# masafumiendo/benchnav

Hardware: AMD Instinct MI355X
Metric: MPPI solve-steps/sec (K=1024,T=50,256x256 map) (higher is better)
Workload: dtype f32

## Files before the change

### benchnav_amd/csrc/rollout_sampled.hip

```cpp
#include "mppi_device.h"

namespace bn {

namespace {

constexpr int kSampledWaves = 8;
constexpr int kSampledThreads = 64 * kSampledWaves;

__host__ __device__ inline size_t sampled_lds_floats(int T, int WN)
{
    const size_t TP = (size_t)((T + 2) & ~1);
    return 4 * 64 * (size_t)(T + 1) + 2 * (size_t)WN * WN + 2 * 64 * TP + 2 * (size_t)T * kUPad + 4 * (size_t)T + 128;
}

template <int EPS, int GEO, bool STORE_U>
__global__ __launch_bounds__(kSampledThreads) void rollout_sampled_kernel(const SolveParams p)
{
    extern __shared__ __attribute__((aligned(16))) float smem[];
    const int T = p.T, K = p.K, WN2 = p.WN * p.WN;
    const int TP = (T + 2) & ~1;
    float4 *XL = reinterpret_cast<float4 *>(smem);
    float2 *win2 = reinterpret_cast<float2 *>(smem + 4 * 64 * (T + 1));
    float *Zt = reinterpret_cast<float *>(win2 + WN2), *Zc = Zt + 64 * TP;
    float *Ul = Zc + 64 * TP, *ml = Ul + 2 * T * kUPad, *mv = ml + 2 * T, *el = mv + 2 * T, *ad = el + 64;
    const WgId wg = decode_wg(p);
    if (wg.idle) return;
    const int tid = threadIdx.x, lane = tid & 63, b = wg.b;
    if (wg.aux) {
        if (p.overlap) finish_body<GEO, true, kSampledThreads, false, true>(p, b, nullptr, p.cost_prev, p.state_prev, smem);
        else finish_body<GEO, true, kSampledThreads>(p, b, nullptr, p.cost_prev, p.state_prev, smem);
        return;
    }
    const int wid = __builtin_amdgcn_readfirstlane(tid >> 6);
    const int k = wg.blk * 64 + lane;
    const bool active = k < K;
    const int kk = active ? k : K - 1;
    const float *__restrict__ mu = p.map + (size_t)b * p.map_stride;
    const float *__restrict__ sg = p.slip_std + (size_t)b * p.map_stride;
    const float sx = p.state[b * 3 + 0], sy = p.state[b * 3 + 1], sth = p.state[b * 3 + 2];
    const float gx = p.goal[b * 2 + 0], gy = p.goal[b * 2 + 1];
    const Win w = window_origin<GEO>(p, sx, sy);
    const size_t Kp = (size_t)p.Kp;
    float *Xb = p.X + (size_t)b * (T + 1) * 3 * Kp + k;
    float *Ub = STORE_U ? p.U + (size_t)b * T * 2 * Kp + k : nullptr;

    BN_STAMP(0);
    for (int e = tid; e < WN2; e += kSampledThreads) {
        const int r = e / p.WN, c = e - r * p.WN;
        const size_t g = (size_t)min(w.wy0 + r, p.G - 1) * p.G + min(w.wx0 + c, p.G - 1);
        win2[e] = make_float2(mu[g], sg[g]);
    }
    const bool ovs = p.overlap != 0;
    const bool tpub = p.flag_part != nullptr;
    if (!ovs)
    for (int j = tid; j < 2 * T; j += kSampledThreads) {
        const float m = p.mean[(size_t)b * 2 * T + j];
        ml[j] = m;
        mv[j] = m * ((j & 1) ? p.iv1 : p.iv0);
    }
    if (wg.blk == 0 && tid < 3) { if (tpub) store_agent(p.state_copy + b * 3 + tid, p.state[b * 3 + tid]); else p.state_copy[b * 3 + tid] = p.state[b * 3 + tid]; }
    if (p.state_snap && wg.blk == 0 && tid < 3) p.state_snap[b * 3 + tid] = p.state[b * 3 + tid];
    __syncthreads();

    {
        const int nE = (T + 1) >> 1, nS = TP >> 1;
        for (int q = nE + wid; q < nE + nS; q += kSampledWaves) {
            {
                const int r0 = 2 * (q - nE), r1 = r0 + 1;
                float z[4];
                if (p.zt) {
                    z[0] = r0 < T ? p.zt[((size_t)b * T + r0) * K + kk] : 0.0f;
                    z[1] = r1 < T ? p.zt[((size_t)b * T + r1) * K + kk] : 0.0f;
                    z[2] = r0 <= T ? p.zc[((size_t)b * (T + 1) + r0) * K + kk] : 0.0f;
                    z[3] = r1 <= T ? p.zc[((size_t)b * (T + 1) + r1) * K + kk] : 0.0f;
                } else {
                    philox_slip_block(p.seed, p.solve, (uint32_t)b, (uint32_t)(kk + p.k0), (uint32_t)(q - nE), z);
                }
                Zt[r0 * 64 + lane] = z[0]; Zt[r1 * 64 + lane] = z[1];
                Zc[r0 * 64 + lane] = z[2]; Zc[r1 * 64 + lane] = z[3];
            }
        }
        if (ovs) {
            if (tid == 0) wait_counter<16>(flag_ctr(p.flag_part, p.prev_slot * p.B + b), p.wait_part, p);
            __syncthreads();
            for (int j = tid; j < 2 * T; j += kSampledThreads) {
                const float m = load_agent(p.mean + (size_t)b * 2 * T + j);
                ml[j] = m;
                mv[j] = m * ((j & 1) ? p.iv1 : p.iv0);
            }
            __syncthreads();
        }
        if (p.mean_snap && wg.blk == 0 && wid == 0) snapshot_mean(p, b, ml, lane);
        for (int q = wid; q < nE; q += kSampledWaves) produce_pair<EPS, STORE_U>(p, p.eps, b, kk, 2 * q, p.solve, ml, Ul, Ub, Kp, lane);
    }
    __syncthreads();
    BN_STAMP(1);

    if (wid == 0) {
        SlipChain c;
        c.x = sx; c.y = sy; c.th = sth;
        sincos_spec(c.th, c.sn, c.cs);
        c.e = slip_cell_safe<GEO, true>(p, w, sx, sy);
        float xn, yn, tn;
        slip_chain_step<GEO, true>(p, win2, w, c, Ul[lane], Ul[kUPad + lane], Zt[lane], xn, yn, tn);
        XL[lane] = make_float4(xn, yn, tn, __int_as_float(c.e));
        int t = 1;
        for (; t + 4 <= T; t += 4) {
            float uq[4][3];
#pragma unroll
            for (int i = 0; i < 4; ++i) {
                uq[i][0] = Ul[(2 * (t + i)) * kUPad + lane]; uq[i][1] = Ul[(2 * (t + i) + 1) * kUPad + lane];
                uq[i][2] = Zt[(t + i) * 64 + lane];
            }
#pragma unroll
            for (int i = 0; i < 4; ++i) {
                slip_chain_step<GEO, false>(p, win2, w, c, uq[i][0], uq[i][1], uq[i][2], xn, yn, tn);
                __builtin_amdgcn_sched_barrier(0);
                XL[(t + i) * 64 + lane] = make_float4(xn, yn, tn, __int_as_float(c.e));
            }
        }
        for (; t < T; ++t) {
            slip_chain_step<GEO, false>(p, win2, w, c, Ul[(2 * t) * kUPad + lane], Ul[(2 * t + 1) * kUPad + lane], Zt[t * 64 + lane],
                                        xn, yn, tn);
            XL[t * 64 + lane] = make_float4(xn, yn, tn, __int_as_float(c.e));
        }
        XL[T * 64 + lane] = make_float4(c.x, c.y, c.th, __int_as_float(c.e));
    } else if (wid == 1) {
        double Ad = 0.0;
        for (int t = 0; t < T; ++t)
            Ad += (double)(p.lambda_ * (mv[2 * t] * Ul[(2 * t) * kUPad + lane] + mv[2 * t + 1] * Ul[(2 * t + 1) * kUPad + lane]));
        ad[lane] = (float)Ad;
    }
    __syncthreads();
    BN_STAMP(2);

    for (int t = wid; t <= T; t += kSampledWaves) {
        const float4 o = XL[t * 64 + lane];
        float *Xt = Xb + (size_t)(3 * t) * Kp;
        Xt[0] = o.x; Xt[Kp] = o.y; Xt[2 * Kp] = o.z;
        const float2 ms = win2[__float_as_int(o.w)];
        const float tc = trav_from_slip(ms.x, ms.y, Zc[t * 64 + lane]);
        const float dx = o.x - gx, dy = o.y - gy;
        Zc[t * 64 + lane] = sqrt_cr_normal(dx * dx + dy * dy) + (tc <= p.thr ? 1.0e4f : 0.0f);
    }
    __syncthreads();
    BN_STAMP(3);

    if (wid == 0) {
        double Sd = 0.0;
#pragma unroll 16
        for (int t = 0; t < T; ++t) Sd += (double)Zc[t * 64 + lane];
        const float cost = ((float)Sd + Zc[T * 64 + lane]) + ad[lane];
        if (active) { if (tpub) store_agent(p.cost + (size_t)b * K + k, cost); else p.cost[(size_t)b * K + k] = cost; }
        const float zz = active ? (-cost) / p.lambda_ : -INFINITY;
        const float zmax = wave_max(zz);
        const float e = active ? expf(zz - zmax) : 0.0f;
        const float esum = wave_sum(e);
        el[lane] = e;
        if (lane == 0) {
            float *part = p.part + ((size_t)b * p.nblk + wg.blk) * (2 + 2 * T);
            store_agent(part, zmax); store_agent(part + 1, esum);
        }
    }
    __syncthreads();
    column_sums<kSampledThreads, true>(Ul, el, T, tid, p.part + ((size_t)b * p.nblk + wg.blk) * (2 + 2 * T));
    BN_STAMP(5);
    if (p.ustar_cur) ticket_merge<kSampledThreads>(p, b, wg.blk, smem);
}

template <int EPS, int GEO, bool STORE_U>
__global__ __launch_bounds__(64) void rollout_sampled_global_kernel(const SolveParams p)
{
    extern __shared__ __attribute__((aligned(16))) float smem[];
    const int T = p.T, K = p.K;
    float *ml = smem, *mv = ml + 2 * T, *Ul = mv + 2 * T, *el = Ul + 2 * T * kUPad;
    const WgId wg = decode_wg(p);
    if (wg.idle) return;
    const int lane = threadIdx.x, b = wg.b;
    const int k = wg.blk * 64 + lane;
    const bool active = k < K;
    const int kk = active ? k : K - 1;
    const float *__restrict__ mu = p.map + (size_t)b * p.map_stride;
    const float *__restrict__ sg = p.slip_std + (size_t)b * p.map_stride;
    const float sx = p.state[b * 3 + 0], sy = p.state[b * 3 + 1], sth = p.state[b * 3 + 2];
    const float gx = p.goal[b * 2 + 0], gy = p.goal[b * 2 + 1];
    const Win w{0, 0, 0.f, 0.f, 0.f, 0.f};
    for (int j = lane; j < 2 * T; j += 64) {
        const float m = p.mean[(size_t)b * 2 * T + j];
        ml[j] = m;
        mv[j] = m * ((j & 1) ? p.iv1 : p.iv0);
    }
    if (wg.blk == 0 && lane < 3) p.state_copy[b * 3 + lane] = p.state[b * 3 + lane];
    if (p.state_snap && wg.blk == 0 && lane < 3) p.state_snap[b * 3 + lane] = p.state[b * 3 + lane];
    __syncthreads();
    const size_t Kp = (size_t)p.Kp;
    float *Xb = p.X + (size_t)b * (T + 1) * 3 * Kp + k;
    float *Ub = STORE_U ? p.U + (size_t)b * T * 2 * Kp + k : nullptr;
    for (int t = 0; t < T; t += 2) produce_pair<EPS, STORE_U>(p, p.eps, b, kk, t, p.solve, ml, Ul, Ub, Kp, lane);
    __syncthreads();
    float x = sx, y = sy, th = sth;
    float sn, cs;
    sincos_spec(th, sn, cs);
    float zq[4] = {0.f, 0.f, 0.f, 0.f};
    double Sd = 0.0, Ad = 0.0;
    for (int t = 0; t < T; ++t) {
        if (p.zt) {
            zq[t & 1] = p.zt[((size_t)b * T + t) * K + kk];
            zq[2 + (t & 1)] = p.zc[((size_t)b * (T + 1) + t) * K + kk];
        } else if ((t & 1) == 0) {
            philox_slip_block(p.seed, p.solve, (uint32_t)b, (uint32_t)(kk + p.k0), (uint32_t)(t >> 1), zq);
        }
        const float u0 = Ul[(2 * t) * kUPad + lane], u1 = Ul[(2 * t + 1) * kUPad + lane];
        const int e = slip_cell_safe<GEO, false>(p, w, x, y);
        const float trav = trav_from_slip(mu[e], sg[e], zq[t & 1]);
        float xn, yn, tn;
        if (p.ref_order) {
            sincos_spec(th, sn, cs);
            const float tv = trav * u0;
            xn = x + (tv * cs) * p.dt; yn = y + (tv * sn) * p.dt;
            tn = th + (trav * u1) * p.dt;
            th = wrap_angle(tn);
        } else {
            const float g = u0 * p.dt, dth = trav * (u1 * p.dt);
            xn = __builtin_fmaf(trav, g * cs, x); yn = __builtin_fmaf(trav, g * sn, y);
            tn = theta_step(th, dth, t == 0);
            rotate_spec(cs, sn, dth);
        }
        float *Xt = Xb + (size_t)(3 * t) * Kp;
        Xt[0] = xn; Xt[Kp] = yn; Xt[2 * Kp] = tn;
        x = clampf(xn, p.x0, p.x_hi); y = clampf(yn, p.y0, p.y_hi);
        const int ec = slip_cell_safe<GEO, false>(p, w, xn, yn);
        const float tc = trav_from_slip(mu[ec], sg[ec], zq[2 + (t & 1)]);
        const float dx = xn - gx, dy = yn - gy;
        Sd += (double)(sqrt_cr_normal(dx * dx + dy * dy) + (tc <= p.thr ? 1.0e4f : 0.0f));
        Ad += (double)(p.lambda_ * (mv[2 * t] * u0 + mv[2 * t + 1] * u1));
    }
    {
        float *Xt = Xb + (size_t)(3 * T) * Kp;
        Xt[0] = x; Xt[Kp] = y; Xt[2 * Kp] = th;
    }
    if (p.zt) zq[2 + (T & 1)] = p.zc[((size_t)b * (T + 1) + T) * K + kk];
    else if ((T & 1) == 0) philox_slip_block(p.seed, p.solve, (uint32_t)b, (uint32_t)(kk + p.k0), (uint32_t)(T >> 1), zq);
    const int eT = slip_cell_safe<GEO, false>(p, w, x, y);
    const float tT = trav_from_slip(mu[eT], sg[eT], zq[2 + (T & 1)]);
    const float dxT = x - gx, dyT = y - gy;
    const float term = sqrt_cr_normal(dxT * dxT + dyT * dyT) + (tT <= p.thr ? 1.0e4f : 0.0f);
    const float cost = ((float)Sd + term) + (float)Ad;
    if (active) p.cost[(size_t)b * K + k] = cost;
    const float zz = active ? (-cost) / p.lambda_ : -INFINITY;
    const float zmax = wave_max(zz);
    const float e = active ? expf(zz - zmax) : 0.0f;
    const float esum = wave_sum(e);
    el[lane] = e;
    __syncthreads();
    float *part = p.part + ((size_t)b * p.nblk + wg.blk) * (2 + 2 * T);
    column_sums<64, false>(Ul, el, T, lane, part);
    if (lane == 0) { part[0] = zmax; part[1] = esum; }
}

__global__ void philox_slip_kernel(float *__restrict__ zt, float *__restrict__ zc, float *__restrict__ zo, uint64_t seed,
                                   uint64_t solve, int b, int K, int T, int k0)
{
    const int nS = ((T + 2) & ~1) >> 1;
    const size_t tot = (size_t)K * nS;
    for (size_t i = blockIdx.x * (size_t)blockDim.x + threadIdx.x; i < tot; i += (size_t)gridDim.x * blockDim.x) {
        const int k = (int)(i / nS), j = (int)(i - (size_t)k * nS);
        float z[4];
        philox_slip_block(seed, solve, (uint32_t)b, (uint32_t)(k + k0), (uint32_t)j, z);
        for (int s = 0; s < 2; ++s) {
            const int r = 2 * j + s;
            if (r < T) zt[(size_t)k * T + r] = z[s];
            if (r <= T) zc[(size_t)k * (T + 1) + r] = z[2 + s];
        }
    }
    if (blockIdx.x == 0)
        for (int j = threadIdx.x; 4 * j < T; j += blockDim.x) {
            float z[4];
            philox_slip_block(seed, solve, (uint32_t)b, 0xffffffffu, (uint32_t)j, z);
            for (int s = 0; s < 4; ++s)
                if (4 * j + s < T) zo[4 * j + s] = z[s];
        }
}


}

size_t sampled_resident_per_cu(const SolveParams &p)
{
    const size_t need = sizeof(float) * sampled_lds_floats(p.T, p.WN);
    return std::max<size_t>(1, std::min<size_t>(160 * 1024 / std::max<size_t>(need, 1), 32 / kSampledWaves));
}

bool sampled_fused(const SolveParams &p)
{
    const size_t need = sizeof(float) * sampled_lds_floats(p.T, p.WN);
    const size_t tail = finish_lds_bytes(p) + sizeof(float) * 64;
    return p.slip_on && !p.ref_order && p.WN > 0 && need <= 160 * 1024 && tail <= need && p.nblk <= 1024;
}


namespace {

template <int EPS, int GEO>
hipError_t launch_sampled_g(const SolveParams &p, hipStream_t s)
{
    const size_t lds_w = sizeof(float) * sampled_lds_floats(p.T, p.WN);
    const dim3 grid = rollout_grid(p, sampled_fused(p) && p.have_prev);
    if (sampled_fused(p)) {
#define BN_SL(SU)                                                                                                      \
    do { hipError_t e = ensure_lds(rollout_sampled_kernel<EPS, GEO, SU>, lds_w); if (e != hipSuccess) return e;        \
         rollout_sampled_kernel<EPS, GEO, SU><<<grid, dim3(kSampledThreads), lds_w, s>>>(p); } while (0)
        if (p.U) BN_SL(true); else BN_SL(false);
#undef BN_SL
    } else {
        const size_t lds = sizeof(float) * (4 * (size_t)p.T + 2 * (size_t)p.T * kUPad + 64);
#define BN_SL(SU)                                                                                                      \
    do { hipError_t e = ensure_lds(rollout_sampled_global_kernel<EPS, GEO, SU>, lds); if (e != hipSuccess) return e;   \
         rollout_sampled_global_kernel<EPS, GEO, SU><<<grid, dim3(64), lds, s>>>(p); } while (0)
        if (p.U) BN_SL(true); else BN_SL(false);
#undef BN_SL
    }
    return hipGetLastError();
}

template <int EPS>
hipError_t launch_sampled_e(const SolveParams &p, hipStream_t s)
{
    switch (geo_of(p)) {
    case kGeoPow2Origin0: return launch_sampled_g<EPS, kGeoPow2Origin0>(p, s);
    case kGeoPow2: return launch_sampled_g<EPS, kGeoPow2>(p, s);
    default: return launch_sampled_g<EPS, kGeoGeneral>(p, s);
    }
}


}

hipError_t launch_rollout_sampled(const SolveParams &p, EpsMode mode, hipStream_t s)
{
    switch (mode) {
    case kEpsPhilox: return launch_sampled_e<kEpsPhilox>(p, s);
    case kEpsKT2: return launch_sampled_e<kEpsKT2>(p, s);
    default: return launch_sampled_e<kEpsT2K>(p, s);
    }
}

hipError_t launch_philox_slip(float *zt, float *zc, float *zo, uint64_t seed, uint64_t solve, int b, int K, int T, int k0, hipStream_t s)
{
    philox_slip_kernel<<<grid_for((size_t)K * (T / 2 + 1)), 256, 0, s>>>(zt, zc, zo, seed, solve, b, K, T, k0);
    return hipGetLastError();
}


}
```

Baseline: 105,800.

## Pipeline sampled rollout stages with LDS progress flags instead of block barriers

Replaces the barrier-separated phases of the sampled rollout kernel with wave-specialized producer/consumer pipelining. Progress counters live in LDS: control chunks are computed in parallel and published, the serial slip chain starts as soon as its first chunk is ready, and other waves stream X writes and per-step cost accumulation behind the chain rather than waiting for it to finish. Noise generation is also split from the mean-dependent clamp, so it can proceed before the overlap wait for the new mean. This shortens the critical path around the serial chain but adds spin-waiting, volatile LDS polling and fragile memory ordering.

```diff
diff --git a/benchnav_amd/csrc/rollout_sampled.hip b/benchnav_amd/csrc/rollout_sampled.hip
--- a/benchnav_amd/csrc/rollout_sampled.hip
+++ b/benchnav_amd/csrc/rollout_sampled.hip
@@ -6,6 +6,33 @@
 
 constexpr int kSampledWaves = 8;
 constexpr int kSampledThreads = 64 * kSampledWaves;
+constexpr int kSampledTail = 4;
+
+typedef __attribute__((address_space(3))) volatile int lds_vint;
+
+__device__ __forceinline__ void post_progress(int *word, int v)
+{
+    asm volatile("" ::: "memory");
+    if ((threadIdx.x & 63) == 0) *(lds_vint *)word = v;
+}
+template <int SLEEP>
+__device__ __forceinline__ int wait_progress(int *word, int need)
+{
+    lds_vint *p3 = (lds_vint *)word;
+    int v;
+    while ((v = *p3) < need) __builtin_amdgcn_s_sleep(SLEEP);
+    asm volatile("" ::: "memory");
+    return __builtin_amdgcn_readfirstlane(v);
+}
+constexpr int kSampledProducers = kSampledWaves - 1;
+__device__ __forceinline__ bool controls_complete(int *prog, int nchunk, int lane)
+{
+    const int w = lane & (kSampledWaves - 1);
+    const int last = w == 0 ? 1 : w < nchunk ? w + ((nchunk - 1 - w) / kSampledProducers) * kSampledProducers + 1 : 0;
+    const int v = *(lds_vint *)(prog + 8 + w);
+    asm volatile("" ::: "memory");
+    return __builtin_amdgcn_ballot_w64(v < last) == 0;
+}
 
 __host__ __device__ inline size_t sampled_lds_floats(int T, int WN)
 {
@@ -23,6 +50,7 @@
     float2 *win2 = reinterpret_cast<float2 *>(smem + 4 * 64 * (T + 1));
     float *Zt = reinterpret_cast<float *>(win2 + WN2), *Zc = Zt + 64 * TP;
     float *Ul = Zc + 64 * TP, *ml = Ul + 2 * T * kUPad, *mv = ml + 2 * T, *el = mv + 2 * T, *ad = el + 64;
+    int *prog = reinterpret_cast<int *>(Zt + 64 * T);
     const WgId wg = decode_wg(p);
     if (wg.idle) return;
     const int tid = threadIdx.x, lane = tid & 63, b = wg.b;
@@ -60,13 +88,16 @@
     }
     if (wg.blk == 0 && tid < 3) { if (tpub) store_agent(p.state_copy + b * 3 + tid, p.state[b * 3 + tid]); else p.state_copy[b * 3 + tid] = p.state[b * 3 + tid]; }
     if (p.state_snap && wg.blk == 0 && tid < 3) p.state_snap[b * 3 + tid] = p.state[b * 3 + tid];
-    __syncthreads();
-
+    if (tid < 8 + kSampledWaves) prog[tid] = 0;
+    __syncthreads();
+
+    const int nchunk = (T + 3) >> 2;
+    const int cstep = wid == 0 ? nchunk : kSampledProducers;
     {
-        const int nE = (T + 1) >> 1, nS = TP >> 1;
-        for (int q = nE + wid; q < nE + nS; q += kSampledWaves) {
+        const int nS = TP >> 1;
+        for (int q = kSampledWaves - 1 - wid; q < nS; q += kSampledWaves) {
             {
-                const int r0 = 2 * (q - nE), r1 = r0 + 1;
+                const int r0 = 2 * q, r1 = r0 + 1;
                 float z[4];
                 if (p.zt) {
                     z[0] = r0 < T ? p.zt[((size_t)b * T + r0) * K + kk] : 0.0f;
@@ -74,27 +105,58 @@
                     z[2] = r0 <= T ? p.zc[((size_t)b * (T + 1) + r0) * K + kk] : 0.0f;
                     z[3] = r1 <= T ? p.zc[((size_t)b * (T + 1) + r1) * K + kk] : 0.0f;
                 } else {
-                    philox_slip_block(p.seed, p.solve, (uint32_t)b, (uint32_t)(kk + p.k0), (uint32_t)(q - nE), z);
+                    philox_slip_block(p.seed, p.solve, (uint32_t)b, (uint32_t)(kk + p.k0), (uint32_t)q, z);
                 }
-                Zt[r0 * 64 + lane] = z[0]; Zt[r1 * 64 + lane] = z[1];
+                if (r0 < T) Zt[r0 * 64 + lane] = z[0];
+                if (r1 < T) Zt[r1 * 64 + lane] = z[1];
                 Zc[r0 * 64 + lane] = z[2]; Zc[r1 * 64 + lane] = z[3];
             }
         }
+        for (int c = wid; c < nchunk; c += cstep)
+            for (int t = 4 * c; t < min(4 * c + 4, T); t += 2) {
+                float e[4];
+                noise_pair<EPS>(p, b, kk, t, e);
+                Ul[(2 * t) * kUPad + lane] = e[0];
+                Ul[(2 * t + 1) * kUPad + lane] = e[1];
+                if (t + 1 < T) { Ul[(2 * t + 2) * kUPad + lane] = e[2]; Ul[(2 * t + 3) * kUPad + lane] = e[3]; }
+            }
         if (ovs) {
             if (tid == 0) wait_counter<16>(flag_ctr(p.flag_part, p.prev_slot * p.B + b), p.wait_part, p);
+            BN_STAMP(13);
             __syncthreads();
             for (int j = tid; j < 2 * T; j += kSampledThreads) {
                 const float m = load_agent(p.mean + (size_t)b * 2 * T + j);
                 ml[j] = m;
                 mv[j] = m * ((j & 1) ? p.iv1 : p.iv0);
             }
-            __syncthreads();
-        }
-        if (p.mean_snap && wg.blk == 0 && wid == 0) snapshot_mean(p, b, ml, lane);
-        for (int q = wid; q < nE; q += kSampledWaves) produce_pair<EPS, STORE_U>(p, p.eps, b, kk, 2 * q, p.solve, ml, Ul, Ub, Kp, lane);
+        }
     }
     __syncthreads();
     BN_STAMP(1);
+
+    for (int c = wid; c < nchunk; c += cstep) {
+        const int t0 = 4 * c;
+        if (t0 + 4 <= T) {
+            float z[8], m[8];
+#pragma unroll
+            for (int i = 0; i < 8; ++i) { z[i] = Ul[(2 * t0 + i) * kUPad + lane]; m[i] = ml[2 * t0 + i]; }
+#pragma unroll
+            for (int i = 0; i < 8; ++i) {
+                const float u = (i & 1) ? clampf(m[i] + p.sigma1 * z[i], p.umin1, p.umax1) : clampf(m[i] + p.sigma0 * z[i], p.umin0, p.umax0);
+                Ul[(2 * t0 + i) * kUPad + lane] = u;
+                if (STORE_U) Ub[(size_t)(2 * t0 + i) * Kp] = u;
+            }
+        } else {
+            for (int t = t0; t < T; ++t) {
+                const float u0 = clampf(ml[2 * t] + p.sigma0 * Ul[(2 * t) * kUPad + lane], p.umin0, p.umax0);
+                const float u1 = clampf(ml[2 * t + 1] + p.sigma1 * Ul[(2 * t + 1) * kUPad + lane], p.umin1, p.umax1);
+                Ul[(2 * t) * kUPad + lane] = u0;
+                Ul[(2 * t + 1) * kUPad + lane] = u1;
+                if (STORE_U) { float *Ut = Ub + (size_t)(2 * t) * Kp; Ut[0] = u0; Ut[Kp] = u1; }
+            }
+        }
+        post_progress(prog + 8 + wid, c + 1);
+    }
 
     if (wid == 0) {
         SlipChain c;
@@ -102,55 +164,97 @@
         sincos_spec(c.th, c.sn, c.cs);
         c.e = slip_cell_safe<GEO, true>(p, w, sx, sy);
         float xn, yn, tn;
+        BN_WSTAMP(0);
+        bool all = controls_complete(prog, nchunk, lane);
         slip_chain_step<GEO, true>(p, win2, w, c, Ul[lane], Ul[kUPad + lane], Zt[lane], xn, yn, tn);
         XL[lane] = make_float4(xn, yn, tn, __int_as_float(c.e));
+        while (!all) { all = controls_complete(prog, nchunk, lane); if (!all) __builtin_amdgcn_s_sleep(1); }
         int t = 1;
-        for (; t + 4 <= T; t += 4) {
-            float uq[4][3];
-#pragma unroll
-            for (int i = 0; i < 4; ++i) {
-                uq[i][0] = Ul[(2 * (t + i)) * kUPad + lane]; uq[i][1] = Ul[(2 * (t + i) + 1) * kUPad + lane];
-                uq[i][2] = Zt[(t + i) * 64 + lane];
-            }
-#pragma unroll
-            for (int i = 0; i < 4; ++i) {
-                slip_chain_step<GEO, false>(p, win2, w, c, uq[i][0], uq[i][1], uq[i][2], xn, yn, tn);
-                __builtin_amdgcn_sched_barrier(0);
-                XL[(t + i) * 64 + lane] = make_float4(xn, yn, tn, __int_as_float(c.e));
-            }
-        }
+#define BN_SCHUNK(POSTALL)                                                                                             \
+        {                                                                                                              \
+            float uq[4][3];                                                                                            \
+            _Pragma("unroll") for (int i = 0; i < 4; ++i) {                                                            \
+                uq[i][0] = Ul[(2 * (t + i)) * kUPad + lane]; uq[i][1] = Ul[(2 * (t + i) + 1) * kUPad + lane];          \
+                uq[i][2] = Zt[(t + i) * 64 + lane];                                                                    \
+            }                                                                                                          \
+            _Pragma("unroll") for (int i = 0; i < 4; ++i) {                                                            \
+                slip_chain_step<GEO, false>(p, win2, w, c, uq[i][0], uq[i][1], uq[i][2], xn, yn, tn);                  \
+                __builtin_amdgcn_sched_barrier(0);                                                                     \
+                XL[(t + i) * 64 + lane] = make_float4(xn, yn, tn, __int_as_float(c.e));                                \
+                if ((POSTALL) || i == 3) post_progress(prog, t + i + 1);                                               \
+            }                                                                                                          \
+        }
+        for (; t + 4 <= T - kSampledTail; t += 4) BN_SCHUNK(false)
+        for (; t + 4 <= T; t += 4) BN_SCHUNK(true)
+#undef BN_SCHUNK
         for (; t < T; ++t) {
             slip_chain_step<GEO, false>(p, win2, w, c, Ul[(2 * t) * kUPad + lane], Ul[(2 * t + 1) * kUPad + lane], Zt[t * 64 + lane],
                                         xn, yn, tn);
             XL[t * 64 + lane] = make_float4(xn, yn, tn, __int_as_float(c.e));
+            post_progress(prog, t + 1);
         }
         XL[T * 64 + lane] = make_float4(c.x, c.y, c.th, __int_as_float(c.e));
+        post_progress(prog, T + 1);
+        BN_STAMP(2);
     } else if (wid == 1) {
+        while (!controls_complete(prog, nchunk, lane)) __builtin_amdgcn_s_sleep(1);
         double Ad = 0.0;
         for (int t = 0; t < T; ++t)
             Ad += (double)(p.lambda_ * (mv[2 * t] * Ul[(2 * t) * kUPad + lane] + mv[2 * t + 1] * Ul[(2 * t + 1) * kUPad + lane]));
         ad[lane] = (float)Ad;
-    }
-    __syncthreads();
-    BN_STAMP(2);
-
-    for (int t = wid; t <= T; t += kSampledWaves) {
-        const float4 o = XL[t * 64 + lane];
-        float *Xt = Xb + (size_t)(3 * t) * Kp;
-        Xt[0] = o.x; Xt[Kp] = o.y; Xt[2 * Kp] = o.z;
-        const float2 ms = win2[__float_as_int(o.w)];
-        const float tc = trav_from_slip(ms.x, ms.y, Zc[t * 64 + lane]);
-        const float dx = o.x - gx, dy = o.y - gy;
-        Zc[t * 64 + lane] = sqrt_cr_normal(dx * dx + dy * dy) + (tc <= p.thr ? 1.0e4f : 0.0f);
-    }
-    __syncthreads();
-    BN_STAMP(3);
-
-    if (wid == 0) {
+        post_progress(prog + 1, 1);
+    } else if (wid == 4) {
+        if (p.mean_snap && wg.blk == 0) snapshot_mean(p, b, ml, lane);
+    } else if (wid != 5) {
+        const int sw = (wid & 1) | ((wid >> 2) << 1);
+        int have = 0;
+        for (int t0 = 4 * sw; t0 <= T; t0 += 16) {
+            const int n = min(4, T + 1 - t0);
+            if (have < t0 + n) have = wait_progress<2>(prog, t0 + n);
+            float *Xt = Xb + (size_t)(3 * t0) * Kp;
+            if (n == 4) {
+                float4 o[4];
+#pragma unroll
+                for (int i = 0; i < 4; ++i) o[i] = XL[(t0 + i) * 64 + lane];
+#pragma unroll
+                for (int i = 0; i < 4; ++i) { Xt[(size_t)(3 * i) * Kp] = o[i].x; Xt[(size_t)(3 * i + 1) * Kp] = o[i].y; Xt[(size_t)(3 * i + 2) * Kp] = o[i].z; }
+            } else {
+                for (int i = 0; i < n; ++i) {
+                    const float4 o = XL[(t0 + i) * 64 + lane];
+                    Xt[(size_t)(3 * i) * Kp] = o.x; Xt[(size_t)(3 * i + 1) * Kp] = o.y; Xt[(size_t)(3 * i + 2) * Kp] = o.z;
+                }
+            }
+        }
+    } else {
+        auto stage = [&](const float4 o, const float z) {
+            const float2 ms = win2[__float_as_int(o.w)];
+            const float tc = trav_from_slip(ms.x, ms.y, z);
+            const float dx = o.x - gx, dy = o.y - gy;
+            return sqrt_cr_normal(dx * dx + dy * dy) + (tc <= p.thr ? 1.0e4f : 0.0f);
+        };
         double Sd = 0.0;
-#pragma unroll 16
-        for (int t = 0; t < T; ++t) Sd += (double)Zc[t * 64 + lane];
-        const float cost = ((float)Sd + Zc[T * 64 + lane]) + ad[lane];
+        float term = 0.0f;
+        int done = 0;
+        while (done <= T) {
+            const int have = wait_progress<1>(prog, done + 1);
+            for (; done + 4 <= min(have, T); done += 4) {
+                float4 o[4];
+                float z[4], s[4];
+#pragma unroll
+                for (int i = 0; i < 4; ++i) { o[i] = XL[(done + i) * 64 + lane]; z[i] = Zc[(done + i) * 64 + lane]; }
+#pragma unroll
+                for (int i = 0; i < 4; ++i) s[i] = stage(o[i], z[i]);
+#pragma unroll
+                for (int i = 0; i < 4; ++i) Sd += (double)s[i];
+            }
+            for (; done < have; ++done) {
+                const float s = stage(XL[done * 64 + lane], Zc[done * 64 + lane]);
+                if (done < T) Sd += (double)s; else term = s;
+            }
+        }
+        wait_progress<1>(prog + 1, 1);
+        BN_WSTAMP(2);
+        const float cost = ((float)Sd + term) + ad[lane];
         if (active) { if (tpub) store_agent(p.cost + (size_t)b * K + k, cost); else p.cost[(size_t)b * K + k] = cost; }
         const float zz = active ? (-cost) / p.lambda_ : -INFINITY;
         const float zmax = wave_max(zz);
@@ -161,8 +265,10 @@
             float *part = p.part + ((size_t)b * p.nblk + wg.blk) * (2 + 2 * T);
             store_agent(part, zmax); store_agent(part + 1, esum);
         }
-    }
-    __syncthreads();
+        BN_WSTAMP(3);
+    }
+    __syncthreads();
+    BN_STAMP(3);
     column_sums<kSampledThreads, true>(Ul, el, T, tid, p.part + ((size_t)b * p.nblk + wg.blk) * (2 + 2 * T));
     BN_STAMP(5);
     if (p.ustar_cur) ticket_merge<kSampledThreads>(p, b, wg.blk, smem);
```

Measured after the change: 104,600. 1.2% lower.
